# bharatlytics/faceRecognition_InfrenceEngine

Hardware: AMD Instinct MI355X
Metric: faces/sec end-to-end @1080p (higher is better)
Workload: dtype f16

## Files before the change

### facerecognition_infrenceengine_amd/csrc/detect_math.h

```cpp
#pragma once
#include "common.h"

struct Lerp { int i0, i1; float w; };

__device__ __forceinline__ Lerp lerp_coord(int d, float ratio, int n) {
    float f = ((float)d + 0.5f) * ratio - 0.5f;
    float fl = floorf(f);
    Lerp r;
    r.w = f - fl;
    int i = (int)fl;
    r.i0 = min(max(i, 0), n - 1);
    r.i1 = min(max(i + 1, 0), n - 1);
    return r;
}

__device__ __forceinline__ float bilerp(float p00, float p01, float p10, float p11, float wx, float wy) {
    float top = (1.0f - wx) * p00 + wx * p01;
    float bot = (1.0f - wx) * p10 + wx * p11;
    return (1.0f - wy) * top + wy * bot;
}

template <class V>
__device__ __forceinline__ void split_f16(float x, V& hi, V& lo, int e) {
    const half_t h = (half_t)x;
    hi[e] = h; lo[e] = (half_t)(x - (float)h);
}

__device__ __forceinline__ bool split_nonfinite(float d) { return !__builtin_isfinite(d); }

__device__ __forceinline__ half_t split_f16_plane(float x, int p) {
    half_t hi[1], lo[1];
    split_f16(x, hi, lo, 0);
    return p ? lo[0] : hi[0];
}
```

### facerecognition_infrenceengine_amd/csrc/pnet_conv1.hip

```cpp
#include "detect_math.h"

namespace {

struct P1Args {
    const uint8_t* frames; int B, FH, FW;
    int H, W;
    const float* w;
    const float* bias; const float* slope;
    float* y;
    unsigned char* y_split;
    int Ho, Wo, Hp, Wp, regions_x, regions_y;
    const int32_t* list; const int32_t* list_count; int list_cap;
};

constexpr int P1_TW = 64, P1_IW = P1_TW + 2;
constexpr int P1_OCC = 3;
constexpr int P1_CTU = 4;
constexpr int P1_LEVEL_SHIFT = 27, P1_TILE_MASK = (1 << P1_LEVEL_SHIFT) - 1;

__device__ __forceinline__ float dpp_xor1(float v) {
    return __int_as_float(__builtin_amdgcn_update_dpp(0, __float_as_int(v), 0xB1, 0xf, 0xf, true));
}
__device__ __forceinline__ float dpp_shr1(float v) {
    return __int_as_float(__builtin_amdgcn_update_dpp(0, __float_as_int(v), 0x111, 0xf, 0xf, true));
}

__device__ __forceinline__ float opaque_inf() {
    float r;
    asm("v_mov_b32 %0, 0x7f800000" : "=v"(r));
    return r;
}
__device__ __forceinline__ float vmax(float x, float y, float pinf) { return __builtin_amdgcn_fmed3f(x, y, pinf); }

template <int RPW, int RPB, bool F16, bool LIST>
__device__ __forceinline__ void pnet_conv1_body(const P1Args& a, const int item0, const int nitems) {
    constexpr int TH = 4 * RPW, IH = TH + 2, NPX = IH * P1_IW;
    constexpr int NPF = (NPX + 255) / 256;
    constexpr int NTAB = IH + P1_IW;
    constexpr int XPX = NPF * 256;
    static_assert(!F16 || XPX >= NPX + P1_IW + 4, "slack behind the tile for the zero-weight taps");
    constexpr int NXB = RPB > 1 ? 2 : 1, NTB = RPB > 1 ? 3 : 1;
    constexpr int XFL = F16 ? XPX * 4 : XPX * 3;
    __shared__ __attribute__((aligned(16))) float xin2[NXB][XFL];
    __shared__ __attribute__((aligned(16))) int4v tab[NTB][NTAB];
    const int tid = threadIdx.x, lane = tid & 63, wave = tid >> 6;
    const float pinf = opaque_inf();

    float wreg[6];
    half8 wfh[2], wfl[2];
    if constexpr (F16) {
#pragma unroll
        for (int st = 0; st < 2; ++st)
#pragma unroll
            for (int j = 0; j < 8; ++j) {
                const int kq_ = lane >> 4, kh = 2 * st + (kq_ >> 1), kw = (kq_ & 1) * 2 + (j >> 2), c = j & 3;
                const float w = (kh < 3 && kw < 3 && c < 3) ? a.w[((kh * 3 + kw) * 4 + c) * 16 + (lane & 15)] : 0.f;
                split_f16(w, wfh[st], wfl[st], j);
            }
    } else {
#pragma unroll
    for (int v = 0; v < 6; ++v) {
        const int c = v * 16 + (lane >> 2), r = lane & 3;
        float x = 0.f;
        if (c < 81) {
            const int k = c / 3, g = c - k * 3, tap = k / 3, ch = k - tap * 3;
            x = a.w[(tap * 4 + ch) * 16 + g * 4 + r];
        }
        wreg[v] = x;
    }
    }

    const int per_img = a.regions_x * a.regions_y;
    auto tile_of = [&](int item) { return LIST ? a.list[item] & P1_TILE_MASK : item; };
    const float ryr = (float)a.FH / (float)a.H, rxr = (float)a.FW / (float)a.W;
    const int frame_bytes = a.FH * a.FW * 3;

    auto make_tables = [&](int item, int buf) __attribute__((always_inline)) {
        if (tid < NTAB) {
            const int tile = tile_of(item);
            const int n = tile / per_img, rem = tile - n * per_img;
            const int ry = rem / a.regions_x, rx = rem - ry * a.regions_x;
            int4v e;
            if (tid < IH) {
                const int yy = ry * TH + tid;
                const Lerp l = lerp_coord(yy, ryr, a.FH);
                e = int4v{l.i0 * a.FW * 3, l.i1 * a.FW * 3, __float_as_int(l.w), yy < a.H ? 1 : 0};
            } else {
                const int xx = rx * P1_TW + (tid - IH);
                const Lerp l = lerp_coord(xx, rxr, a.FW);
                e = int4v{l.i0 * 3, __float_as_int(l.w), l.i1 != l.i0 ? 1 : 0, xx < a.W ? 1 : 0};
            }
            tab[buf][tid] = e;
        }
    };

    unsigned long long rq0[NPF], rq1[NPF];
    int rfl[NPF];
    int pos[NPF];
#pragma unroll
    for (int u = 0; u < NPF; ++u) {
        const int e = min(tid + u * 256, NPX - 1), iy = e / P1_IW;
        pos[u] = iy | ((IH + e - iy * P1_IW) << 16);
    }
    bool edge = true;
    auto load_tile = [&](int item, int buf) __attribute__((always_inline)) {
        const int n = tile_of(item) / per_img;
        const uint8_t* fbase = a.frames + (int64_t)n * frame_bytes;
        const bool last = n == a.B - 1;
        const int lim = frame_bytes - 8;
        int4v re[NPF], ce[NPF];
        bool special = false;
#pragma unroll
        for (int u = 0; u < NPF; ++u) { re[u] = tab[buf][pos[u] & 0xffff]; ce[u] = tab[buf][pos[u] >> 16]; }
#pragma unroll
        for (int u = 0; u < NPF; ++u) {
// ... 431 lines not shown
```

### facerecognition_infrenceengine_amd/csrc/ro_conv1.hip

```cpp
#include "detect_math.h"

constexpr int RC1_PB_R = 3;
constexpr int RC1_RPB_R = 16;
constexpr int RC1_PB_O = 2;
constexpr int RC1_RPB_O = 4;

namespace {

struct RoArgs {
    const uint8_t* frames; int nframes, H, W;
    const float* boxes; const int32_t* counts; int cap;
    const float* w;
    const float* bias; const float* slope;
    float* y;
    unsigned char* ys;
    const int32_t* list; const int32_t* list_count; int list_cap;
};

__device__ __forceinline__ float vmax_r(float x, float y) {
    float r;
    asm("v_max_f32 %0, %1, %2" : "=v"(r) : "v"(x), "v"(y));
    return r;
}

template <int S, int NG, int COUT, int PB, int RPB, bool SPLIT = false, bool LIST = false, bool F16 = false>
__global__ __launch_bounds__(256) void crop_conv1_kernel(RoArgs a) {
    constexpr int C = S - 2;
    constexpr int P = (C - 3 + 1) / 2 + 1;
    constexpr int CS = (NG * 4) % 32 ? NG * 4 : NG * 4 + 4;
    constexpr int BR = 2 * PB + 1 < C ? 2 * PB + 1 : C;
    constexpr int NBAND = (P + PB - 1) / PB;
    constexpr int NPF = (S * S + 255) / 256;
    static_assert(NG * 4 <= 32 && COUT <= NG * 4, "cout quads");
    constexpr int NW = (27 * NG + 15) / 16;
    constexpr int XPX = S * S + S + 8;
    constexpr int XFLOATS = F16 ? (2 * XPX * 8 / 4 + 3) & ~3 : (S * S * 3 + 3) & ~3;
    extern __shared__ __attribute__((aligned(16))) float lds_ro[];
    float* xin = lds_ro;
    int4v* tab = reinterpret_cast<int4v*>(lds_ro + XFLOATS);
    float4* sbox_mem = reinterpret_cast<float4*>(tab + 4 * S);
    int* sorig = reinterpret_cast<int*>(sbox_mem + RPB);
    float* ot = reinterpret_cast<float*>(sorig + ((RPB + 3) & ~3));
    const int tid = threadIdx.x, lane = tid & 63, wave = tid >> 6;
    const int s_first = blockIdx.x * RPB;
    int s_end;
    if constexpr (LIST) {
        s_end = min(s_first + RPB, min(*a.list_count, a.list_cap));
    } else {
        const int fblk = s_first / a.cap;
        s_end = min(s_first + RPB, fblk * a.cap + a.counts[fblk]);
    }
    int slot = s_first;
    if (slot >= s_end) return;
    auto next_valid = [&](int s) { return s < s_end ? s : -1; };
    float4* sbox = sbox_mem;
    if (tid < s_end - s_first) {
        const int o = LIST ? a.list[s_first + tid] : s_first + tid;
        sorig[tid] = o;
        sbox[tid] = *reinterpret_cast<const float4*>(a.boxes + (int64_t)o * 4);
    }
    __syncthreads();
    float wreg[F16 ? 1 : NW];
    half8 wfh[F16 ? 2 : 1][2], wfl[F16 ? 2 : 1][2];
    if constexpr (F16) {
        unsigned char* xz = reinterpret_cast<unsigned char*>(xin);
        for (int e = tid; e < (S + 8) * 2; e += 256)
            *reinterpret_cast<unsigned long long*>(xz + ((e & 1) * XPX + S * S + (e >> 1)) * 8) = 0ull;
        const int li_ = lane & 15, kq_ = lane >> 4;
#pragma unroll
        for (int st = 0; st < 2; ++st)
#pragma unroll
            for (int ct = 0; ct < 2; ++ct)
#pragma unroll
                for (int j = 0; j < 8; ++j) {
                    const int kh = 2 * st + (kq_ >> 1), kw = (kq_ & 1) * 2 + (j >> 2), c = j & 3, co = ct * 16 + li_;
                    const float w = (kh < 3 && kw < 3 && c < 3 && co < NG * 4) ? a.w[((kh * 3 + kw) * 3 + c) * (NG * 4) + co] : 0.f;
                    split_f16(w, wfh[st][ct], wfl[st][ct], j);
                }
    } else {
#pragma unroll
    for (int v = 0; v < NW; ++v) {
        const int c = v * 16 + (lane >> 2), r = lane & 3;
        wreg[v] = c < 27 * NG ? a.w[(c / NG) * (NG * 4) + (c % NG) * 4 + r] : 0.f;
    }
    }
    bool mono = true;
    for (int c = 0; c < NG * 4; ++c) mono = mono && a.slope[c] >= 0.f;

    unsigned long long rq0[NPF], rq1[NPF];
    int rfl[NPF];
    bool edge = true;
    auto make_tab = [&](int sl, int buf) __attribute__((always_inline)) {
        if (tid < 2 * S) {
            const float4 b = sbox[sl - s_first];
            const int x1 = (int)truncf(b.x), y1 = (int)truncf(b.y), x2 = (int)truncf(b.z), y2 = (int)truncf(b.w);
            const int tw = x2 - x1 + 1, th = y2 - y1 + 1;
            int4v e = {0, 0, 0, 0};
            if (tw > 0 && th > 0) {
                if (tid < S) {
                    const Lerp l = lerp_coord(tid, (float)th / (float)S, th);
                    e = int4v{y1 - 1 + l.i0, y1 - 1 + l.i1, __float_as_int(l.w), 1};
                } else {
                    const Lerp l = lerp_coord(tid - S, (float)tw / (float)S, tw);
                    e = int4v{x1 - 1 + l.i0, x1 - 1 + l.i1, __float_as_int(l.w), 1};
                }
            }
            tab[buf * 2 * S + tid] = e;
        }
    };
    auto load_crop = [&](int sl, int buf) __attribute__((always_inline)) {
        const int f = sorig[sl - s_first] / a.cap;
        const uint8_t* fr = a.frames + (int64_t)f * a.H * a.W * 3;
        const int lim = f == a.nframes - 1 ? a.H * a.W * 3 - 8 : 0x7fffffff;
        bool special = false;
#pragma unroll
        for (int u = 0; u < NPF; ++u) {
            const int t = min(tid + u * 256, S * S - 1);
            const int oy = t / S, ox = t - oy * S;
            const int4v re = tab[buf * 2 * S + oy], ce = tab[buf * 2 * S + S + ox];
            rq0[u] = rq1[u] = 0; rfl[u] = -1;
            if (re[3]) {
                const int xs0 = ce[0], xs1 = ce[1];
                const bool in0 = xs0 >= 0 && xs0 < a.W, in1 = xs1 >= 0 && xs1 < a.W;
                const int basecol = in0 ? xs0 : xs1;
                const int src0 = in0 ? 1 : 0;
                const int src1 = in1 ? (xs1 == basecol ? 1 : 2) : 0;
                int fl = src0 | (src1 << 2);
                if (src0 | src1) {
#pragma unroll
                    for (int r = 0; r < 2; ++r) {
                        const int ys = r ? re[1] : re[0];
                        if (ys >= 0 && ys < a.H) {
                            const int off = (ys * a.W + basecol) * 3;
                            const int c8 = min(off, lim);
                            const unsigned long long q = *reinterpret_cast<const u64_unaligned*>(fr + c8);
                            if (r) rq1[u] = q; else rq0[u] = q;
                            fl |= ((off - c8) * 8) << (8 + 8 * r);
                        }
                    }
                }
                rfl[u] = fl;
                special = special || fl != (1 | (2 << 2));
            }
        }
        edge = __builtin_amdgcn_ballot_w64(special) != 0;
    };
    auto store_crop_as = [&](int buf, auto EDGE) __attribute__((always_inline)) {
        constexpr bool E = decltype(EDGE)::value;
#pragma unroll
        for (int u = 0; u < NPF; ++u) {
            const int t = tid + u * 256;
            if (t >= S * S) continue;
            const int oy = t / S, ox = t - oy * S;
            const float wy = __int_as_float(tab[buf * 2 * S + oy][2]), wx = __int_as_float(tab[buf * 2 * S + S + ox][2]);
            float v[3] = {0.f, 0.f, 0.f};
            if (rfl[u] >= 0) {
                const unsigned long long q0 = E ? rq0[u] >> ((rfl[u] >> 8) & 0xff) : rq0[u];
                const unsigned long long q1 = E ? rq1[u] >> ((rfl[u] >> 16) & 0xff) : rq1[u];
                const unsigned l0 = (unsigned)q0, h0 = (unsigned)(q0 >> 32), l1 = (unsigned)q1, h1 = (unsigned)(q1 >> 32);
                const float f0[3] = {(float)((l0 >> 16) & 0xff), (float)((l0 >> 8) & 0xff), (float)(l0 & 0xff)};
                const float s0[3] = {(float)((h0 >> 8) & 0xff), (float)(h0 & 0xff), (float)(l0 >> 24)};
                const float f1[3] = {(float)((l1 >> 16) & 0xff), (float)((l1 >> 8) & 0xff), (float)(l1 & 0xff)};
                const float s1[3] = {(float)((h1 >> 8) & 0xff), (float)(h1 & 0xff), (float)(l1 >> 24)};
                const int src0 = rfl[u] & 3, src1 = (rfl[u] >> 2) & 3;
#pragma unroll
                for (int ch = 0; ch < 3; ++ch) {
                    const float p00 = E ? (src0 ? f0[ch] : 0.f) : f0[ch], p10 = E ? (src0 ? f1[ch] : 0.f) : f1[ch];
                    const float p01 = E ? (src1 == 2 ? s0[ch] : (src1 == 1 ? f0[ch] : 0.f)) : s0[ch];
                    const float p11 = E ? (src1 == 2 ? s1[ch] : (src1 == 1 ? f1[ch] : 0.f)) : s1[ch];
                    v[ch] = __builtin_fmaf(bilerp(p00, p01, p10, p11, wx, wy), 0.0078125f, -0.99609375f);
                }
            }
            if constexpr (F16) {
                half4 hi, lo;
#pragma unroll
                for (int ch = 0; ch < 3; ++ch) split_f16(v[ch], hi, lo, ch);
                hi[3] = lo[3] = (half_t)0.f;
                unsigned char* xz = reinterpret_cast<unsigned char*>(xin);
                *reinterpret_cast<half4*>(xz + t * 8) = hi;
                *reinterpret_cast<half4*>(xz + (XPX + t) * 8) = lo;
            } else {
                xin[t * 3 + 0] = v[0]; xin[t * 3 + 1] = v[1]; xin[t * 3 + 2] = v[2];
            }
        }
    };

    make_tab(slot, 0);
    __syncthreads();
    load_crop(slot, 0);
    for (int buf = 0; slot >= 0; buf ^= 1) {
    const int nslot = next_valid(slot + 1);
    if (edge) store_crop_as(buf, std::true_type{});
    else store_crop_as(buf, std::false_type{});
    if (nslot >= 0) make_tab(nslot, buf ^ 1);
    __syncthreads();
    if (nslot >= 0) load_crop(nslot, buf ^ 1);

    float* yo = a.y + (int64_t)slot * P * P * COUT;
    for (int band = 0; band < NBAND; ++band) {
        const int r0 = band * 2 * PB;
        const int nrow = min(BR, C - r0);
        const int npx = nrow * C;
        if constexpr (F16) {
            typedef half8 half8_a8 __attribute__((aligned(8)));
            const unsigned char* xz = reinterpret_cast<const unsigned char*>(xin);
            const int li_ = lane & 15, kq_ = lane >> 4;
            for (int tl = wave; tl * 16 < npx; tl += 4) {
                const int pidx = min(tl * 16 + li_, npx - 1);
                const int ly = pidx / C, lx = pidx - ly * C;
                const unsigned char* pb = xz + ((r0 + ly + (kq_ >> 1)) * S + lx + 2 * (kq_ & 1)) * 8;
                const half8 h0 = *reinterpret_cast<const half8_a8*>(pb), l0 = *reinterpret_cast<const half8_a8*>(pb + XPX * 8);
                const half8 h1 = *reinterpret_cast<const half8_a8*>(pb + 2 * S * 8), l1 = *reinterpret_cast<const half8_a8*>(pb + (XPX + 2 * S) * 8);
                float4v acc[2];
#pragma unroll
                for (int ct = 0; ct < 2; ++ct) {
                    float4v d = {0.f, 0.f, 0.f, 0.f};
                    d = __builtin_amdgcn_mfma_f32_16x16x32_f16(wfl[0][ct], h0, d, 0, 0, 0);
                    d = __builtin_amdgcn_mfma_f32_16x16x32_f16(wfh[0][ct], l0, d, 0, 0, 0);
                    d = __builtin_amdgcn_mfma_f32_16x16x32_f16(wfl[1][ct], h1, d, 0, 0, 0);
                    d = __builtin_amdgcn_mfma_f32_16x16x32_f16(wfh[1][ct], l1, d, 0, 0, 0);
                    d = __builtin_amdgcn_mfma_f32_16x16x32_f16(wfh[0][ct], h0, d, 0, 0, 0);
                    d = __builtin_amdgcn_mfma_f32_16x16x32_f16(wfh[1][ct], h1, d, 0, 0, 0);
                    acc[ct] = d;
                }
                if (tl * 16 + li_ < npx) {
                    float* o = ot + (tl * 16 + li_) * CS;
#pragma unroll
                    for (int ct = 0; ct < 2; ++ct) {
                        const int co = ct * 16 + 4 * kq_;
                        if (co < NG * 4) {
                            float4v v = acc[ct];
                            if (!mono) {
                                v += *reinterpret_cast<const float4v*>(a.bias + co);
                                const float4v sv = *reinterpret_cast<const float4v*>(a.slope + co);
#pragma unroll
                                for (int e = 0; e < 4; ++e) v[e] = v[e] > 0.f ? v[e] : v[e] * sv[e];
                            }
                            *reinterpret_cast<float4v*>(o + co) = v;
                        }
                    }
                }
            }
        } else
        for (int u = wave; u * 64 < npx; u += 4) {
            const int pidx = min(u * 64 + lane, npx - 1);
            const int ly = pidx / C, lx = pidx - ly * C;
            const float* xb = xin + ((r0 + ly) * S + lx) * 3;
            float4v acc[NG];
#pragma unroll
            for (int g = 0; g < NG; ++g) acc[g] = float4v{0.f, 0.f, 0.f, 0.f};
            static_for<27>([&](auto K) {
                constexpr int k = decltype(K)::value;
                constexpr int kh = k / 9, q = k - kh * 9;
                const float xv = xb[kh * S * 3 + q];
                static_for<NG>([&](auto G) {
                    constexpr int g = decltype(G)::value;
                    constexpr int c = k * NG + g;
                    acc[g] = __builtin_amdgcn_mfma_f32_4x4x1f32(wreg[c / 16], xv, acc[g], 4, c % 16, 0);
                });
            });
            if (u * 64 + lane < npx) {
                float* o = ot + (u * 64 + lane) * CS;
#pragma unroll
                for (int g = 0; g < NG; ++g) {
                    float4v v = acc[g];
                    if (!mono) {
                        v += *reinterpret_cast<const float4v*>(a.bias + g * 4);
                        const float4v sv = *reinterpret_cast<const float4v*>(a.slope + g * 4);
#pragma unroll
                        for (int e = 0; e < 4; ++e) v[e] = v[e] > 0.f ? v[e] : v[e] * sv[e];
                    }
                    *reinterpret_cast<float4v*>(o + g * 4) = v;
                }
            }
        }
        __syncthreads();
        const int p0 = band * PB;
        const int prow = min(PB, P - p0);
        constexpr int Q4 = COUT / 4;
        for (int e = tid; e < prow * P * Q4; e += 256) {
            const int qd = e % Q4, pp = e / Q4;
            const int pyl = pp / P, px = pp - pyl * P;
            float4v m = {-INFINITY, -INFINITY, -INFINITY, -INFINITY};
#pragma unroll
            for (int dy = 0; dy < 3; ++dy) {
                const int ry = min(2 * pyl + dy, nrow - 1);
#pragma unroll
                for (int dx = 0; dx < 3; ++dx) {
                    const int cx = min(2 * px + dx, C - 1);
                    const float4v v = *reinterpret_cast<const float4v*>(ot + (ry * C + cx) * CS + qd * 4);
#pragma unroll
                    for (int k = 0; k < 4; ++k) m[k] = vmax_r(m[k], v[k]);
                }
            }
            if (mono) {
                m += *reinterpret_cast<const float4v*>(a.bias + qd * 4);
                const float4v sv = *reinterpret_cast<const float4v*>(a.slope + qd * 4);
#pragma unroll
                for (int k = 0; k < 4; ++k) m[k] = m[k] > 0.f ? m[k] : m[k] * sv[k];
            }
            if constexpr (SPLIT) {
                half4 hi, lo;
#pragma unroll
                for (int k = 0; k < 4; ++k) split_f16(m[k], hi, lo, k);
                unsigned char* o2 = a.ys + ((int64_t)slot * P * P + (p0 + pyl) * P + px) * 128 + qd * 8;
                *reinterpret_cast<half4*>(o2) = hi;
                *reinterpret_cast<half4*>(o2 + 64) = lo;
                if constexpr (COUT < 32) {
                    if (qd == Q4 - 1) {
#pragma unroll
                        for (int z = COUT / 4; z < 8; ++z) {
                            *reinterpret_cast<half4*>(o2 + (z - qd) * 8) = half4{0, 0, 0, 0};
                            *reinterpret_cast<half4*>(o2 + 64 + (z - qd) * 8) = half4{0, 0, 0, 0};
                        }
                    }
                }
            } else {
                *reinterpret_cast<float4v*>(yo + ((int64_t)(p0 + pyl) * P + px) * COUT + qd * 4) = m;
            }
        }
        if (band + 1 < NBAND) __syncthreads();
    }
    __syncthreads();
    slot = nslot;
    }
}

template <int S, int NG, int COUT, int PB, int RPB, bool SPLIT = false, bool LIST = false, bool F16 = false>
int launch_ro(const RoArgs& a, int nslots, hipStream_t s) {
    constexpr int C = S - 2;
    constexpr int rows = 2 * PB + 1 < C ? 2 * PB + 1 : C;
    constexpr int CS = (NG * 4) % 32 ? NG * 4 : NG * 4 + 4;
    constexpr int XFLOATS = F16 ? (2 * (S * S + S + 8) * 8 / 4 + 3) & ~3 : (S * S * 3 + 3) & ~3;
    const size_t lds = (size_t)(XFLOATS + 4 * S * 4 + RPB * 4 + ((RPB + 3) & ~3) + rows * C * CS) * sizeof(float);
    auto kern = crop_conv1_kernel<S, NG, COUT, PB, RPB, SPLIT, LIST, F16>;
    if (lds > 64 * 1024) {
        static FrDevLatch latch;
        if (!fr_raise_lds(reinterpret_cast<const void*>(kern), lds, latch)) {
            fr_set_error("fr_crop_conv1_f32: cannot raise dynamic LDS to %zu bytes", lds);
            return FR_E_LAUNCH;
        }
    }
    kern<<<(nslots + RPB - 1) / RPB, 256, lds, s>>>(a);
    return FR_OK;
}

}

extern "C" int fr_crop_conv1_f32(int net, const uint8_t* frames, int nframes, int H, int W, const float* boxes,
                                 const int32_t* counts, int cap, const float* w, const float* bias, const float* slope,
                                 float* y, fr_stream_t stream) {
    FR_REQUIRE(frames && boxes && counts && w && bias && slope && y, "fr_crop_conv1_f32: null pointer");
    FR_REQUIRE(nframes > 0 && cap > 0 && H > 0 && W > 0 && (int64_t)H * W * 3 < (1ll << 31) && (int64_t)H * W * 3 >= 8,
               "fr_crop_conv1_f32: bad frame size");
    FR_REQUIRE((int64_t)nframes * cap < (1ll << 31), "fr_crop_conv1_f32: too many slots");
    RoArgs a{frames, nframes, H, W, boxes, counts, cap, w, bias, slope, y, nullptr, nullptr, nullptr, 0};
    int rc;
    hipStream_t s = fr_stream(stream);
    const int64_t nslots = (int64_t)nframes * cap;
    if (net == 0) rc = cap % 8 == 0 && nslots >= 8192 ? launch_ro<24, 7, 28, 4, 8>(a, nframes * cap, s) : launch_ro<24, 7, 28, 4, 1>(a, nframes * cap, s);
    else if (net == 1) rc = cap % 4 == 0 && nslots >= 2048 ? launch_ro<48, 8, 32, 2, 4>(a, nframes * cap, s) : launch_ro<48, 8, 32, 2, 1>(a, nframes * cap, s);
    else { FR_REQUIRE(false, "fr_crop_conv1_f32: net must be 0 (R-Net) or 1 (O-Net)"); }
    if (rc != FR_OK) return rc;
    FR_CHECK_LAUNCH("crop_conv1_kernel");
    return FR_OK;
}

extern "C" int fr_crop_conv1_split(int net, const uint8_t* frames, int nframes, int H, int W, const float* boxes,
                                   const int32_t* counts, int cap, const float* w, const float* bias, const float* slope,
                                   void* y_split, int conv_f16, fr_stream_t stream) {
    FR_REQUIRE(frames && boxes && counts && w && bias && slope && y_split, "fr_crop_conv1_split: null pointer");
    FR_REQUIRE(nframes > 0 && cap > 0 && H > 0 && W > 0 && (int64_t)H * W * 3 < (1ll << 31) && (int64_t)H * W * 3 >= 8,
               "fr_crop_conv1_split: bad frame size");
    FR_REQUIRE((int64_t)nframes * cap < (1ll << 31), "fr_crop_conv1_split: too many slots");
    RoArgs a{frames, nframes, H, W, boxes, counts, cap, w, bias, slope, nullptr, (unsigned char*)y_split, nullptr, nullptr, 0};
    hipStream_t s = fr_stream(stream);
    const int64_t nslots = (int64_t)nframes * cap;
    int rc;
    if (conv_f16) {
        if (net == 0) rc = cap % RC1_RPB_R == 0 && nslots >= 8192 ? launch_ro<24, 7, 28, RC1_PB_R, RC1_RPB_R, true, false, true>(a, nframes * cap, s) : launch_ro<24, 7, 28, 4, 1, true, false, true>(a, nframes * cap, s);
        else if (net == 1) rc = cap % RC1_RPB_O == 0 && nslots >= 2048 ? launch_ro<48, 8, 32, RC1_PB_O, RC1_RPB_O, true, false, true>(a, nframes * cap, s) : launch_ro<48, 8, 32, 2, 1, true, false, true>(a, nframes * cap, s);
        else { FR_REQUIRE(false, "fr_crop_conv1_split: net must be 0 (R-Net) or 1 (O-Net)"); }
    } else
    if (net == 0) rc = cap % 8 == 0 && nslots >= 8192 ? launch_ro<24, 7, 28, 4, 8, true>(a, nframes * cap, s) : launch_ro<24, 7, 28, 4, 1, true>(a, nframes * cap, s);
    else if (net == 1) rc = cap % 4 == 0 && nslots >= 2048 ? launch_ro<48, 8, 32, 2, 4, true>(a, nframes * cap, s) : launch_ro<48, 8, 32, 2, 1, true>(a, nframes * cap, s);
    else { FR_REQUIRE(false, "fr_crop_conv1_split: net must be 0 (R-Net) or 1 (O-Net)"); }
    if (rc != FR_OK) return rc;
    FR_CHECK_LAUNCH("crop_conv1_kernel (split)");
    return FR_OK;
}

extern "C" int fr_crop_conv1_list_f32(int net, const uint8_t* frames, int nframes, int H, int W, const float* boxes, int cap,
                                      const int32_t* list, const int32_t* list_count, int list_cap, const float* w,
                                      const float* bias, const float* slope, float* y, fr_stream_t stream) {
    FR_REQUIRE(frames && boxes && list && list_count && w && bias && slope && y, "fr_crop_conv1_list_f32: null pointer");
    FR_REQUIRE(nframes > 0 && cap > 0 && list_cap > 0 && H > 0 && W > 0 && (int64_t)H * W * 3 < (1ll << 31) && (int64_t)H * W * 3 >= 8,
               "fr_crop_conv1_list_f32: bad argument");
    RoArgs a{frames, nframes, H, W, boxes, nullptr, cap, w, bias, slope, y, nullptr, list, list_count, list_cap};
    hipStream_t s = fr_stream(stream);
    int rc;
    if (net == 0) rc = launch_ro<24, 7, 28, 4, 1, false, true>(a, list_cap, s);
    else if (net == 1) rc = launch_ro<48, 8, 32, 2, 1, false, true>(a, list_cap, s);
    else { FR_REQUIRE(false, "fr_crop_conv1_list_f32: net must be 0 (R-Net) or 1 (O-Net)"); }
    if (rc != FR_OK) return rc;
    FR_CHECK_LAUNCH("crop_conv1_kernel (list)");
    return FR_OK;
}
```

### include/frhip.h

```cpp
#ifndef FRHIP_H
#define FRHIP_H
#include <stddef.h>
#include <stdint.h>
#ifdef __cplusplus
extern "C" {
#endif

#define FR_OK 0
#define FR_E_INVALID (-1)
#define FR_E_LAUNCH (-2)
#define FR_E_NODEVICE (-3)

typedef void* fr_stream_t;

#define FR_ABI_VERSION 106
int fr_version(void);
const char* fr_last_error_string(void);
int fr_device_count(void);

int fr_l2norm_rows_f32(const float* x, float* out, int rows, int dim, fr_stream_t stream);

size_t fr_gallery_match_workspace(int F, int64_t N);
int fr_gallery_match_f32(const float* Q, const float* G, int F, int64_t N, int D,
                         int64_t row_offset, int64_t* out_idx, float* out_score,
// ... 112 lines not shown
                               void* workspace, size_t workspace_bytes, fr_stream_t stream);

typedef struct {
    const void* x; const void* w; void* y;
    const float* bias; const float* slope; const void* residual;
    float* out_f32_partial;
    int B, H, W, Cin, Cout, KH, KW, stride, pad, Ho, Wo;
    int bias_mode; int splitk;
    const void* x2; int C2;
} fr_conv_args;
int fr_conv_nhwc_f16(const fr_conv_args* args, fr_stream_t stream);
typedef struct {
    const void* x8; const void* w8; void* y16; void* y8;
    const float* oscale; const float* bias; const float* slope; const void* residual;
    int B, H, W, Cin, Cout, bias_mode;
    float y8_mul;
    const float* y8_sub;
} fr_conv_f8_args;
int fr_conv_nhwc_f8(const fr_conv_f8_args* args, fr_stream_t stream);
int fr_quantize_f16_f8(const void* x16, void* out8, int64_t n, float mul, fr_stream_t stream);
int fr_quantize_f16_f8_centred(const void* x16, void* out8, int64_t n, int C, const float* sub, float mul,
                               fr_stream_t stream);
size_t fr_conv_stage14_weight_bytes(int nconv);
int fr_conv_stage14_pack(const void* w, void* out, fr_stream_t stream);
int fr_conv_stage14_f16(const void* x, void* y, const void* wstream, const float* params, int B, int nblocks,
                        fr_stream_t stream);
size_t fr_conv_stage28_weight_bytes(int nconv);
int fr_conv_stage28_pack(const void* w, void* out, fr_stream_t stream);
int fr_conv_stage28_f16(void* x, void* mid, const void* wstream, const float* params, int B, int nblocks, fr_stream_t stream);
size_t fr_conv_walk64_weight_bytes(int Cout);
int fr_conv_walk64_pack(const void* w, void* out, int Cout, fr_stream_t stream);
int fr_conv_walk64_f16(const void* x, const void* wstream, void* y, const float* bias, int bias_mode, const float* slope,
                       const void* residual, int B, int HW, int Cout, fr_stream_t stream);
size_t fr_conv_stage14_f8_weight_bytes(int nconv);
size_t fr_conv_stage14_f8_param_floats(void);
int fr_conv_stage14_f8_pack(const void* w8, void* out, fr_stream_t stream);
int fr_conv_stage14_f8(const void* x8, const void* x16, void* y16, const void* wstream, const float* params, int B,
                       int nblocks, fr_stream_t stream);
int fr_gptq_round_e4m3(const double* W, const double* U, const float* sw, float* Q, int rows, int K, fr_stream_t stream);
int fr_conv_splitk_epilogue(const float* partial, int splitk, int M, int Cout, int Ho, int Wo,
                            const float* bias, int bias_mode, const float* slope, const void* residual,
                            void* y, fr_stream_t stream);
int fr_conv_inblock_f16(const fr_conv_args* args, fr_stream_t stream);
typedef struct {
    int kind;
    fr_conv_args args;
} fr_conv_step;
int fr_conv_sequence(const fr_conv_step* steps, int nsteps, fr_stream_t stream);
int fr_fc_reduce_l2norm(const float* partial, int splitk, int B, int dim, const float* bias,
                        float* embedding, float* normed, fr_stream_t stream);


int fr_warp_affine_5pt(const uint8_t* frames, int nframes, int H, int W, const float* kps,
                       const int32_t* frame_idx, const int32_t* count, int F, int size,
                       void* out_f16_nhwc8, uint8_t* out_u8_bgr, float* M_out, fr_stream_t stream);

int fr_warp_affine_5pt_slots(const uint8_t* frames, int nframes, int H, int W, const float* kps,
                             const int32_t* counts, int cap, int size, void* out_f16_nhwc8,
                             fr_stream_t stream);

typedef struct {
    const uint8_t* data;
    int32_t H, W, nh, nw;
    int32_t reserved[2];
} fr_frame_ref;
int fr_warp_affine_5pt_refs(const fr_frame_ref* refs, int nframes, const float* kps, const int32_t* frame_idx,
                            const int32_t* count, int F, int size, void* out_f16_nhwc8, uint8_t* out_u8_bgr,
                            float* M_out, fr_stream_t stream);
int fr_warp_affine_5pt_slots_refs(const fr_frame_ref* refs, int nframes, const float* kps, const int32_t* counts,
                                  int cap, int size, void* out_f16_nhwc8, fr_stream_t stream);

int fr_pyramid_resize_norm(const uint8_t* frames, int nframes, int H, int W, int hs, int ws,
                           float* out, fr_stream_t stream);
int fr_dconv_f32(const float* x, const float* w, const float* bias, const float* slope, float* y,
                 int B, int H, int W, int Cin, int Cout, int CoutP, int KH, int KW, int pool2,
                 const float* head_w, const float* head_b, int nhead, fr_stream_t stream);
int fr_dconv_mfma_f32(int layer, const float* x, const float* w, const float* bias, const float* slope,
                      float* y, int B, int H, int W, const float* head_w, const float* head_b,
                      const uint8_t* frames, int FH, int FW, const int32_t* counts, int cap, void* y_split,
                      fr_stream_t stream);
int fr_crop_conv1_f32(int net, const uint8_t* frames, int nframes, int H, int W, const float* boxes,
                      const int32_t* counts, int cap, const float* w, const float* bias, const float* slope,
                      float* y, fr_stream_t stream);
int fr_crop_conv1_split(int net, const uint8_t* frames, int nframes, int H, int W, const float* boxes,
                        const int32_t* counts, int cap, const float* w, const float* bias, const float* slope,
                        void* y_split, int conv_f16, fr_stream_t stream);
int fr_crop_conv1_list_f32(int net, const uint8_t* frames, int nframes, int H, int W, const float* boxes, int cap,
                           const int32_t* list, const int32_t* list_count, int list_cap, const float* w,
                           const float* bias, const float* slope, float* y, fr_stream_t stream);
int fr_ro_conv2_split(int net, const void* x_split, const float* w, const float* bias, const float* slope, float* y,
                      int nslots, const int32_t* counts, int cap, int32_t* zero_word, fr_stream_t stream);
size_t fr_ro_gemm_weight_bytes(int layer);
int fr_ro_gemm_pack(int layer, const float* w, void* out, fr_stream_t stream);
int fr_ro_gemm_split(int layer, const float* x, const void* w_packed, const float* bias, const float* slope, float* y,
                     int nslots, const int32_t* counts, int cap, fr_stream_t stream);
int fr_ro_margin_list(const float* head, int nhead, const int32_t* counts, int nframes, int cap, float logit_thr,
                      float margin, int32_t* list, int32_t* list_count, int list_cap, fr_stream_t stream);
int fr_ro_scatter_rows(const float* src, const int32_t* list, const int32_t* list_count, int list_cap, int ncols,
                       float* dst, fr_stream_t stream);
size_t fr_pnet23_workspace_bytes(int B, int H1, int W1);
int fr_pnet23_split_f16(const float* x1, const void* x1s, int B, int H1, int W1, const float* w2, const float* b2, const float* s2,
                        const float* w3, const float* b3, const float* s3, const float* hw, const float* hb,
                        float* head, int all_heads, float refine_logit_thr, float refine_band_hi, int32_t* refined_count,
                        void* workspace, size_t workspace_bytes, fr_stream_t stream);
size_t fr_pnet23_coarse_workspace_bytes(int B, int H1, int W1);
int fr_pnet23_coarse_f16(const float* x1, const void* x1s, int B, int H1, int W1, const float* w2, const float* b2, const float* s2,
                         const float* w3, const float* b3, const float* s3, const float* hw, const float* hb,
                         float* head, int all_heads, float refine_logit_thr, float refine_band_hi, int32_t* refined_count,
                         void* workspace, size_t workspace_bytes, float coarse_margin, void* coarse, size_t coarse_bytes,
                         int32_t* visited_count, fr_stream_t stream);
int fr_maxpool_f32(const float* x, float* y, int B, int H, int W, int C, int k, int stride,
                   fr_stream_t stream);
int fr_pnet_candidates(const float* head, int nframes, int hc, int wc, float scale, float thr, int cap,
                       float* boxes, float* scores, float* regs, int32_t* counts,
                       int32_t* block_counts, float* prob_out, const float* dl, float dl_min, fr_stream_t stream);
int fr_sort_nms(const float* boxes, const float* scores, const float* aux, int naux,
                const int32_t* counts, int L, int nseg, int seg_cap, int seg_major, float thr, int mode,
                int max_keep,
                float* boxes_out, float* scores_out, float* aux_out, int32_t* counts_out,
                int cap_out, fr_stream_t stream);
int fr_box_refine(float* boxes, const float* aux, int naux, const int32_t* counts, int L, int cap,
                  int mode, fr_stream_t stream);
int fr_crop_resize_norm(const uint8_t* frames, int nframes, int H, int W, const float* boxes,
                        const int32_t* counts, int cap, int size, float* out, fr_stream_t stream);
int fr_stage_select(const float* boxes, const float* head, int nh, const int32_t* counts, int L, int cap,
                    float thr, float* boxes_out, float* scores_out, float* aux_out, int naux,
                    int32_t* counts_out, float* prob_out, fr_stream_t stream);

int fr_pnet_conv1_band(int mode, const uint8_t* frames, int B, int FH, int FW, int H, int W, const float* w, const float* bias,
                       const float* slope, float* y, void* y_split, const int32_t* list, const int32_t* list_count, int list_cap,
                       fr_stream_t stream);
size_t fr_pnet_band_tiles_count(int B, int H1, int W1);
int fr_pnet_band_tiles(const void* workspace, int B, int H1, int W1, int32_t* tbuf, int32_t* tiles, fr_stream_t stream);
typedef struct {
    const float* x1; float* head; void* workspace;
    int H1, W1; float scale;
    float* boxes; float* scores; float* regs; int32_t* counts; int32_t* block_counts;
    void* x1s;
    int hs, ws;
    int f16;
} fr_pnet_level;
int fr_pnet_finish_levels(const fr_pnet_level* levels, int nlevels, int nframes, const float* w2, const float* b2,
                          const float* s2, const float* w3, const float* b3, const float* s3, const float* hw,
                          const float* hb, float thr, int cap, float dl_min, int32_t* refined_count, fr_stream_t stream);
int fr_pnet_pyramid_conv1(int mode, const uint8_t* frames, int B, int FH, int FW, const fr_pnet_level* levels, int nlevels,
                          const float* w, const float* bias, const float* slope, const int32_t* list, const int32_t* list_count,
                          int list_cap, fr_stream_t stream);
int fr_pnet_pyramid_p23(const fr_pnet_level* levels, int nlevels, int nframes, const float* w2, const float* b2, const float* s2,
                        const float* w3, const float* b3, const float* s3, const float* hw, const float* hb, int all_heads,
                        float refine_logit_thr, float refine_band_hi, fr_stream_t stream);
int fr_pnet_pyramid_band_tiles(const fr_pnet_level* levels, int nlevels, int nframes, int32_t* tbuf, int32_t* tiles, fr_stream_t stream);
int fr_pnet_pyramid_p23_coarse(const fr_pnet_level* levels, int nlevels, int nframes, const float* w2, const float* b2, const float* s2,
                               const float* w3, const float* b3, const float* s3, const float* hw, const float* hb, int all_heads,
                               float refine_logit_thr, float refine_band_hi, float coarse_margin, void* const* coarse,
                               int32_t* visited_count, fr_stream_t stream);

int fr_letterbox_u8(const fr_frame_ref* refs, int nframes, uint8_t* canvas, int dh, int dw, fr_stream_t stream);
int fr_detections_unscale(float* boxes, float* kps, const int32_t* counts, const float* det_scale, int nframes, int cap,
                          fr_stream_t stream);

#define FR_YUV_NV12 0
#define FR_YUV_I420 1
int fr_yuv420_to_bgr_u8(const uint8_t* src, uint8_t* dst, int N, int H, int W, int layout, int y_off, int cy, int cub, int cug,
                        int cvg, int cvr, fr_stream_t stream);
int fr_yuv420_to_bgr_refs_u8(const fr_frame_ref* dst_refs, const uint8_t* const* src_ptrs, int nframes, int layout, int y_off,
                             int cy, int cub, int cug, int cvg, int cvr, fr_stream_t stream);
// ... 59 lines not shown
```

Baseline: 26190.

## Add strip-form O-Net conv1 kernel computing rows with fused pooling in registers

Adds a STRIP variant of the O-Net crop conv1 kernel. Each wave handles a column strip and walks rows, doing the MFMA conv, 3x3 max-pool via DPP and row-running max, and the f16 split store directly from registers, with no LDS band buffer and no band syncs. It also uses fewer slots per block and a higher occupancy hint, and adds a batch-shape flag that forces the batched path. The STRIP form is only chosen when conv_f16==1, so whether it runs depends on what the caller passes.

```diff
diff --git a/facerecognition_infrenceengine_amd/csrc/detect_math.h b/facerecognition_infrenceengine_amd/csrc/detect_math.h
--- a/facerecognition_infrenceengine_amd/csrc/detect_math.h
+++ b/facerecognition_infrenceengine_amd/csrc/detect_math.h
@@ -20,6 +20,13 @@
     return (1.0f - wy) * top + wy * bot;
 }
 
+__device__ __forceinline__ float opaque_inf() {
+    float r;
+    asm("v_mov_b32 %0, 0x7f800000" : "=v"(r));
+    return r;
+}
+__device__ __forceinline__ float vmax(float x, float y, float pinf) { return __builtin_amdgcn_fmed3f(x, y, pinf); }
+
 template <class V>
 __device__ __forceinline__ void split_f16(float x, V& hi, V& lo, int e) {
     const half_t h = (half_t)x;
diff --git a/facerecognition_infrenceengine_amd/csrc/pnet_conv1.hip b/facerecognition_infrenceengine_amd/csrc/pnet_conv1.hip
--- a/facerecognition_infrenceengine_amd/csrc/pnet_conv1.hip
+++ b/facerecognition_infrenceengine_amd/csrc/pnet_conv1.hip
@@ -24,13 +24,6 @@
 __device__ __forceinline__ float dpp_shr1(float v) {
     return __int_as_float(__builtin_amdgcn_update_dpp(0, __float_as_int(v), 0x111, 0xf, 0xf, true));
 }
-
-__device__ __forceinline__ float opaque_inf() {
-    float r;
-    asm("v_mov_b32 %0, 0x7f800000" : "=v"(r));
-    return r;
-}
-__device__ __forceinline__ float vmax(float x, float y, float pinf) { return __builtin_amdgcn_fmed3f(x, y, pinf); }
 
 template <int RPW, int RPB, bool F16, bool LIST>
 __device__ __forceinline__ void pnet_conv1_body(const P1Args& a, const int item0, const int nitems) {
diff --git a/facerecognition_infrenceengine_amd/csrc/ro_conv1.hip b/facerecognition_infrenceengine_amd/csrc/ro_conv1.hip
--- a/facerecognition_infrenceengine_amd/csrc/ro_conv1.hip
+++ b/facerecognition_infrenceengine_amd/csrc/ro_conv1.hip
@@ -4,6 +4,8 @@
 constexpr int RC1_RPB_R = 16;
 constexpr int RC1_PB_O = 2;
 constexpr int RC1_RPB_O = 4;
+constexpr int RC1_RPB_OS = 2;
+constexpr int RC1_OCC_OS = 3;
 
 namespace {
 
@@ -23,10 +25,11 @@
     return r;
 }
 
-template <int S, int NG, int COUT, int PB, int RPB, bool SPLIT = false, bool LIST = false, bool F16 = false>
-__global__ __launch_bounds__(256) void crop_conv1_kernel(RoArgs a) {
+template <int S, int NG, int COUT, int PB, int RPB, bool SPLIT = false, bool LIST = false, bool F16 = false, bool STRIP = false>
+__global__ __launch_bounds__(256, STRIP ? RC1_OCC_OS : 1) void crop_conv1_kernel(RoArgs a) {
     constexpr int C = S - 2;
     constexpr int P = (C - 3 + 1) / 2 + 1;
+    static_assert(!STRIP || (F16 && SPLIT && !LIST && (P + 6) / 7 == 4 && C % 2 == 0 && P == C / 2), "strip form");
     constexpr int CS = (NG * 4) % 32 ? NG * 4 : NG * 4 + 4;
     constexpr int BR = 2 * PB + 1 < C ? 2 * PB + 1 : C;
     constexpr int NBAND = (P + PB - 1) / PB;
@@ -35,6 +38,7 @@
     constexpr int NW = (27 * NG + 15) / 16;
     constexpr int XPX = S * S + S + 8;
     constexpr int XFLOATS = F16 ? (2 * XPX * 8 / 4 + 3) & ~3 : (S * S * 3 + 3) & ~3;
+    static_assert(!F16 || (C + 2) * S + C + 3 <= XPX, "slack behind the crop image");
     extern __shared__ __attribute__((aligned(16))) float lds_ro[];
     float* xin = lds_ro;
     int4v* tab = reinterpret_cast<int4v*>(lds_ro + XFLOATS);
@@ -73,7 +77,8 @@
             for (int ct = 0; ct < 2; ++ct)
 #pragma unroll
                 for (int j = 0; j < 8; ++j) {
-                    const int kh = 2 * st + (kq_ >> 1), kw = (kq_ & 1) * 2 + (j >> 2), c = j & 3, co = ct * 16 + li_;
+                    const int kh = 2 * st + (kq_ >> 1), kw = (kq_ & 1) * 2 + (j >> 2), c = j & 3;
+                    const int co = STRIP ? 8 * (li_ >> 2) + 4 * ct + (li_ & 3) : ct * 16 + li_;
                     const float w = (kh < 3 && kw < 3 && c < 3 && co < NG * 4) ? a.w[((kh * 3 + kw) * 3 + c) * (NG * 4) + co] : 0.f;
                     split_f16(w, wfh[st][ct], wfl[st][ct], j);
                 }
@@ -89,6 +94,11 @@
 
     unsigned long long rq0[NPF], rq1[NPF];
     int rfl[NPF];
+    auto strip_tid = [&]() __attribute__((always_inline)) {
+        int t = tid;
+        if constexpr (STRIP) asm volatile("" : "+v"(t));
+        return t;
+    };
     bool edge = true;
     auto make_tab = [&](int sl, int buf) __attribute__((always_inline)) {
         if (tid < 2 * S) {
@@ -113,9 +123,10 @@
         const uint8_t* fr = a.frames + (int64_t)f * a.H * a.W * 3;
         const int lim = f == a.nframes - 1 ? a.H * a.W * 3 - 8 : 0x7fffffff;
         bool special = false;
+        const int tix = strip_tid();
 #pragma unroll
         for (int u = 0; u < NPF; ++u) {
-            const int t = min(tid + u * 256, S * S - 1);
+            const int t = min(tix + u * 256, S * S - 1);
             const int oy = t / S, ox = t - oy * S;
             const int4v re = tab[buf * 2 * S + oy], ce = tab[buf * 2 * S + S + ox];
             rq0[u] = rq1[u] = 0; rfl[u] = -1;
@@ -147,9 +158,10 @@
     };
     auto store_crop_as = [&](int buf, auto EDGE) __attribute__((always_inline)) {
         constexpr bool E = decltype(EDGE)::value;
+        const int tix = strip_tid();
 #pragma unroll
         for (int u = 0; u < NPF; ++u) {
-            const int t = tid + u * 256;
+            const int t = tix + u * 256;
             if (t >= S * S) continue;
             const int oy = t / S, ox = t - oy * S;
             const float wy = __int_as_float(tab[buf * 2 * S + oy][2]), wx = __int_as_float(tab[buf * 2 * S + S + ox][2]);
@@ -196,6 +208,96 @@
     __syncthreads();
     if (nslot >= 0) load_crop(nslot, buf ^ 1);
 
+    if constexpr (STRIP) {
+        typedef half8 half8_a8 __attribute__((aligned(8)));
+        const int li_ = lane & 15, kq_ = lane >> 4, st = wave;
+        const int col = 14 * st + li_;
+        const bool incol = col < C;
+        const unsigned char* pb0 = reinterpret_cast<const unsigned char*>(xin) + ((kq_ >> 1) * S + min(col, C - 1) + 2 * (kq_ & 1)) * 8;
+        const float pinf = opaque_inf();
+        const int px = 7 * st + (li_ >> 1);
+        const bool odd = li_ & 1;
+        const bool emits = li_ < 14 && px < P;
+        unsigned char* os = a.ys + (int64_t)slot * (P * P * 128);
+        const int ol = min(px, P - 1) * 128 + (li_ & 1) * 64 + kq_ * 16;
+        auto quad = [&](const float* q, int ct) __attribute__((always_inline)) {
+            int kq = kq_;
+            asm volatile("" : "+v"(kq));
+            return *reinterpret_cast<const float4v*>(q + min(8 * kq + 4 * ct, NG * 4 - 4));
+        };
+        auto conv_row = [&](int row, auto use) __attribute__((always_inline)) {
+            const unsigned char* pb = pb0 + row * S * 8;
+            const half8 h0 = *reinterpret_cast<const half8_a8*>(pb), l0 = *reinterpret_cast<const half8_a8*>(pb + XPX * 8);
+            const half8 h1 = *reinterpret_cast<const half8_a8*>(pb + 2 * S * 8), l1 = *reinterpret_cast<const half8_a8*>(pb + (XPX + 2 * S) * 8);
+#pragma unroll
+            for (int ct = 0; ct < 2; ++ct) {
+                float4v d = {0.f, 0.f, 0.f, 0.f};
+                d = __builtin_amdgcn_mfma_f32_16x16x32_f16(wfl[0][ct], h0, d, 0, 0, 0);
+                d = __builtin_amdgcn_mfma_f32_16x16x32_f16(wfh[0][ct], l0, d, 0, 0, 0);
+                d = __builtin_amdgcn_mfma_f32_16x16x32_f16(wfl[1][ct], h1, d, 0, 0, 0);
+                d = __builtin_amdgcn_mfma_f32_16x16x32_f16(wfh[1][ct], l1, d, 0, 0, 0);
+                d = __builtin_amdgcn_mfma_f32_16x16x32_f16(wfh[0][ct], h0, d, 0, 0, 0);
+                d = __builtin_amdgcn_mfma_f32_16x16x32_f16(wfh[1][ct], h1, d, 0, 0, 0);
+                if (!mono) {
+                    d += quad(a.bias, ct);
+                    const float4v sv = quad(a.slope, ct);
+#pragma unroll
+                    for (int e = 0; e < 4; ++e) d[e] = d[e] > 0.f ? d[e] : d[e] * sv[e];
+                }
+                float4v h;
+#pragma unroll
+                for (int e = 0; e < 4; ++e) {
+                    const float v = incol ? d[e] : -INFINITY;
+                    float v1 = __int_as_float(__builtin_amdgcn_update_dpp(0, __float_as_int(v), 0x101, 0xf, 0xf, true));
+                    float v2 = __int_as_float(__builtin_amdgcn_update_dpp(0, __float_as_int(v), 0x102, 0xf, 0xf, true));
+                    asm volatile("" : "+v"(v1), "+v"(v2));
+                    h[e] = vmax(vmax(v, v1, pinf), v2, pinf);
+                }
+                use(ct, h);
+            }
+        };
+        auto emit = [&](const float4v (&mx)[2], int prow) __attribute__((always_inline)) {
+            half8 hi, lo;
+#pragma unroll
+            for (int ct = 0; ct < 2; ++ct) {
+                float4v m = mx[ct];
+                if (mono) {
+                    m += quad(a.bias, ct);
+                    const float4v sv = quad(a.slope, ct);
+#pragma unroll
+                    for (int e = 0; e < 4; ++e) m[e] = m[e] > 0.f ? m[e] : m[e] * sv[e];
+                }
+                const bool real = 8 * kq_ + 4 * ct < COUT;
+#pragma unroll
+                for (int e = 0; e < 4; ++e) split_f16(real ? m[e] : 0.f, hi, lo, 4 * ct + e);
+            }
+            const int4v hv = __builtin_bit_cast(int4v, hi), lv = __builtin_bit_cast(int4v, lo);
+            int4v o;
+#pragma unroll
+            for (int e = 0; e < 4; ++e) {
+                int t = __builtin_amdgcn_update_dpp(0, lv[e], 0x111, 0xf, 0xf, true);
+                asm volatile("" : "+v"(t));
+                o[e] = odd ? t : hv[e];
+            }
+            if (emits) *reinterpret_cast<int4v*>(os + (ol + prow * (P * 128))) = o;
+        };
+        auto max4 = [&](float4v x, float4v y) __attribute__((always_inline)) {
+            float4v r;
+#pragma unroll
+            for (int e = 0; e < 4; ++e) r[e] = vmax(x[e], y[e], pinf);
+            return r;
+        };
+        float4v rm[2], t[2];
+        conv_row(0, [&](int ct, float4v h) { rm[ct] = h; });
+        conv_row(1, [&](int ct, float4v h) { rm[ct] = max4(rm[ct], h); });
+#pragma unroll 1
+        for (int rp = 1; rp < C / 2; ++rp) {
+            conv_row(2 * rp, [&](int ct, float4v h) { t[ct] = max4(rm[ct], h); rm[ct] = h; });
+            emit(t, rp - 1);
+            conv_row(2 * rp + 1, [&](int ct, float4v h) { rm[ct] = max4(rm[ct], h); });
+        }
+        emit(rm, P - 1);
+    } else {
     float* yo = a.y + (int64_t)slot * P * P * COUT;
     for (int band = 0; band < NBAND; ++band) {
         const int r0 = band * 2 * PB;
@@ -321,19 +423,20 @@
         }
         if (band + 1 < NBAND) __syncthreads();
     }
+    }
     __syncthreads();
     slot = nslot;
     }
 }
 
-template <int S, int NG, int COUT, int PB, int RPB, bool SPLIT = false, bool LIST = false, bool F16 = false>
+template <int S, int NG, int COUT, int PB, int RPB, bool SPLIT = false, bool LIST = false, bool F16 = false, bool STRIP = false>
 int launch_ro(const RoArgs& a, int nslots, hipStream_t s) {
     constexpr int C = S - 2;
     constexpr int rows = 2 * PB + 1 < C ? 2 * PB + 1 : C;
     constexpr int CS = (NG * 4) % 32 ? NG * 4 : NG * 4 + 4;
     constexpr int XFLOATS = F16 ? (2 * (S * S + S + 8) * 8 / 4 + 3) & ~3 : (S * S * 3 + 3) & ~3;
-    const size_t lds = (size_t)(XFLOATS + 4 * S * 4 + RPB * 4 + ((RPB + 3) & ~3) + rows * C * CS) * sizeof(float);
-    auto kern = crop_conv1_kernel<S, NG, COUT, PB, RPB, SPLIT, LIST, F16>;
+    const size_t lds = (size_t)(XFLOATS + 4 * S * 4 + RPB * 4 + ((RPB + 3) & ~3) + (STRIP ? 0 : rows * C * CS)) * sizeof(float);
+    auto kern = crop_conv1_kernel<S, NG, COUT, PB, RPB, SPLIT, LIST, F16, STRIP>;
     if (lds > 64 * 1024) {
         static FrDevLatch latch;
         if (!fr_raise_lds(reinterpret_cast<const void*>(kern), lds, latch)) {
@@ -377,13 +480,17 @@
     hipStream_t s = fr_stream(stream);
     const int64_t nslots = (int64_t)nframes * cap;
     int rc;
-    if (conv_f16) {
-        if (net == 0) rc = cap % RC1_RPB_R == 0 && nslots >= 8192 ? launch_ro<24, 7, 28, RC1_PB_R, RC1_RPB_R, true, false, true>(a, nframes * cap, s) : launch_ro<24, 7, 28, 4, 1, true, false, true>(a, nframes * cap, s);
-        else if (net == 1) rc = cap % RC1_RPB_O == 0 && nslots >= 2048 ? launch_ro<48, 8, 32, RC1_PB_O, RC1_RPB_O, true, false, true>(a, nframes * cap, s) : launch_ro<48, 8, 32, 2, 1, true, false, true>(a, nframes * cap, s);
+    const int form = conv_f16 & 3;
+    FR_REQUIRE(form < 3 && (conv_f16 & ~(3 | FR_RC1_BATCH_SHAPE)) == 0, "fr_crop_conv1_split: conv_f16 must be 0, 1 or 2 (| 16)");
+    const bool many_r = nslots >= 8192 || (conv_f16 & FR_RC1_BATCH_SHAPE), many_o = nslots >= 2048 || (conv_f16 & FR_RC1_BATCH_SHAPE);
+    if (form) {
+        if (net == 0) rc = cap % RC1_RPB_R == 0 && many_r ? launch_ro<24, 7, 28, RC1_PB_R, RC1_RPB_R, true, false, true>(a, nframes * cap, s) : launch_ro<24, 7, 28, 4, 1, true, false, true>(a, nframes * cap, s);
+        else if (net == 1 && form == 1) rc = cap % RC1_RPB_OS == 0 && many_o ? launch_ro<48, 8, 32, RC1_PB_O, RC1_RPB_OS, true, false, true, true>(a, nframes * cap, s) : launch_ro<48, 8, 32, 2, 1, true, false, true>(a, nframes * cap, s);
+        else if (net == 1) rc = cap % RC1_RPB_O == 0 && many_o ? launch_ro<48, 8, 32, RC1_PB_O, RC1_RPB_O, true, false, true>(a, nframes * cap, s) : launch_ro<48, 8, 32, 2, 1, true, false, true>(a, nframes * cap, s);
         else { FR_REQUIRE(false, "fr_crop_conv1_split: net must be 0 (R-Net) or 1 (O-Net)"); }
     } else
-    if (net == 0) rc = cap % 8 == 0 && nslots >= 8192 ? launch_ro<24, 7, 28, 4, 8, true>(a, nframes * cap, s) : launch_ro<24, 7, 28, 4, 1, true>(a, nframes * cap, s);
-    else if (net == 1) rc = cap % 4 == 0 && nslots >= 2048 ? launch_ro<48, 8, 32, 2, 4, true>(a, nframes * cap, s) : launch_ro<48, 8, 32, 2, 1, true>(a, nframes * cap, s);
+    if (net == 0) rc = cap % 8 == 0 && many_r ? launch_ro<24, 7, 28, 4, 8, true>(a, nframes * cap, s) : launch_ro<24, 7, 28, 4, 1, true>(a, nframes * cap, s);
+    else if (net == 1) rc = cap % 4 == 0 && many_o ? launch_ro<48, 8, 32, 2, 4, true>(a, nframes * cap, s) : launch_ro<48, 8, 32, 2, 1, true>(a, nframes * cap, s);
     else { FR_REQUIRE(false, "fr_crop_conv1_split: net must be 0 (R-Net) or 1 (O-Net)"); }
     if (rc != FR_OK) return rc;
     FR_CHECK_LAUNCH("crop_conv1_kernel (split)");
diff --git a/include/frhip.h b/include/frhip.h
--- a/include/frhip.h
+++ b/include/frhip.h
@@ -218,6 +218,7 @@
 int fr_crop_conv1_f32(int net, const uint8_t* frames, int nframes, int H, int W, const float* boxes,
                       const int32_t* counts, int cap, const float* w, const float* bias, const float* slope,
                       float* y, fr_stream_t stream);
+#define FR_RC1_BATCH_SHAPE 16
 int fr_crop_conv1_split(int net, const uint8_t* frames, int nframes, int H, int W, const float* boxes,
                         const int32_t* counts, int cap, const float* w, const float* bias, const float* slope,
                         void* y_split, int conv_f16, fr_stream_t stream);
```

Result: faster. 26490, median of 6 (+1.1%).
